# the-lay/voltools

Hardware: AMD Instinct MI355X
Metric: Mvoxels/s, 512^3 f32 filt_bspline StaticVolume transform (resident source, device output) (higher is better)
Workload: dtype f32; 1 GPU; 512^3 float32 filt_bspline, StaticVolume resident in HBM, rotate((0,i,0)) rzxz sweep, output= device buffer; lds_bytes=34816, kernel=8, resident_bytes=1660944384, angles=i

## Files before the change

### voltools_amd/csrc/vt_host.h

```cpp
#pragma once
#include "vt_internal.h"
#include "vt_resident.h"

#include <algorithm>
#include <cstdlib>
#include <vector>

struct Tuning {
    int tile = -1;
    int la = 0;
    int march_box = -1;
    int lxpad = -1;
    int dch = 0;
    int blk_h = -1, blk_w = -1;
    bool plain_tile_order = false;
    int rswap_wfast = -1;
    bool exp_nostore = false;
    bool exp_noload = false;
    bool exp_nolds = false;
    bool exp_noloop = false;
    bool exp_stamps = false;
    bool exp_notiles = false;
    bool exp_static = false;
    int quad_rows = -2;
    int quad_grid2d = 1;
    int quad_reverse = -1;
    bool test_fail_copy = false;
    int quad_perm = 1;
    bool no_proj_cache = false;
    int quad_pingpong = 1;
    int quad_zid = 1;
    int reorient = 4;
    int rows_pd = 8;
    int no_fused_relayout = 0;
    int rows_db = 0;
    int rows = 1;
    int quad_zfir = 1;
    int zid_dch = 0;
    int quad_nt = -1;
    bool no_block = false;
    int block_rs = -1;
    bool block_linear = false;
    bool block_no_trim = false;
    int block_min = 240;
    int block_pad = -1;
    double max_resident_gb = 0.0;
    int span = 1;
    int span_pipe = 0;
    int block_th = 8;
    int64_t dot_part_cap = 64ll << 20;
    void read()
    {
        auto num = [](const char* name, int dflt) { const char* e = std::getenv(name); return e ? std::atoi(e) : dflt; };
        tile = num("VT_TILE", -1);
#ifdef VT_LEGACY
        la = num("VT_LA", 0);
        march_box = num("VT_MARCH_BOX", -1);
        if (march_box > 1) march_box = 1;
        lxpad = num("VT_LXPAD", -1);
#endif
        dch = std::max(0, num("VT_DCH", 0));
        blk_h = num("VT_BLK_H", -1);
        blk_w = num("VT_BLK_W", -1);
        plain_tile_order = num("VT_TILE_ORDER", 1) == 0;
        rswap_wfast = num("VT_RSWAP_WFAST", -1);
#ifdef VT_EXPERIMENTS
        exp_nostore = std::getenv("VT_EXP_NOSTORE") != nullptr;
        exp_noload = std::getenv("VT_EXP_NOLOAD") != nullptr;
        exp_nolds = std::getenv("VT_EXP_NOLDS") != nullptr;
        exp_noloop = std::getenv("VT_EXP_NOLOOP") != nullptr;
        exp_static = std::getenv("VT_EXP_STATIC") != nullptr;
        exp_notiles = std::getenv("VT_EXP_NOTILES") != nullptr;
        exp_stamps = std::getenv("VT_EXP_STAMPS") != nullptr;
#endif
        quad_nt = num("VT_QUAD_NT", -1);
#ifdef VT_LEGACY
        test_fail_copy = std::getenv("VT_TEST_FAIL_COPY") != nullptr;
        quad_perm = num("VT_QUAD_PERM", 1);
        quad_zid = num("VT_QUAD_ZID", 1);
        quad_grid2d = num("VT_QUAD_GRID2D", 1);
#endif
        quad_pingpong = num("VT_QUAD_PINGPONG", 1);
        quad_zfir = num("VT_QUAD_ZFIR", 1);
        rows = num("VT_ROWS", 1);
        rows_pd = num("VT_ROWS_PD", 8);
        rows_db = num("VT_ROWS_DB", 0);
        no_fused_relayout = num("VT_NO_FUSED_RELAYOUT", 0);
        reorient = num("VT_REORIENT", 4);
        no_proj_cache = std::getenv("VT_NO_PROJ_CACHE") != nullptr;
        zid_dch = num("VT_ZID_DCH", 0);
        quad_reverse = num("VT_QUAD_REVERSE", -1);
        quad_rows = num("VT_QUAD_ROWS", -2);
        no_block = std::getenv("VT_NO_BLOCK_KERNEL") != nullptr;
        block_rs = num("VT_BLOCK_RS", -1);
        block_linear = std::getenv("VT_BLOCK_LINEAR") != nullptr;
        block_pad = num("VT_BLOCK_PAD", -1);
        block_th = num("VT_BLOCK_TH", 8) == 16 ? 16 : 8;
        span_pipe = num("VT_SPAN_PIPE", 0);
        span = num("VT_SPAN", 1);
        { const char* e = std::getenv("VT_MAX_RESIDENT_GB"); max_resident_gb = e ? std::atof(e) : 0.0; }
        block_min = std::max(1, num("VT_BLOCK_MIN", 240));
        block_no_trim = std::getenv("VT_BLOCK_NO_TRIM") != nullptr;
        { const char* e = std::getenv("VT_DOT_PART_CAP"); if (e && std::atoll(e) > 0) dot_part_cap = std::min<int64_t>(std::atoll(e), 64ll << 20); }
    }
};


struct vt_volume {
    unsigned launch_no = 0;
    int dev = 0;
    int interp = 0;
    int D = 0, H = 0, W = 0;
    int oD = 0, oH = 0, oW = 0;
    int64_t plane0 = 0;
    int64_t gD = 0;
    int64_t out_plane0 = 0;
    int P = 0;
    float* d_src = nullptr;
    size_t src_bytes = 0;
    float* d_zeros = nullptr;
    int Pr = 0;
    int Px = 0;
    int reorient_asked[3] = {0, 0, 0};
    vt::LazyCopies lazy;
    float copies_ms = 0.f;
    int copies_built = 0, copies_evicted = 0;
    hipEvent_t evc0 = nullptr, evc1 = nullptr;
    int* d_queue = nullptr;
    void* d_tplan = nullptr;
    size_t tplan_bytes = 0;
    uint32_t tplan_epoch = 0;
    float* d_scratch_out = nullptr;
    double* d_batch_m = nullptr;
    std::vector<double> h_batch_m;
    size_t batch_m_cap = 0;
    float* d_proj_tmp = nullptr;
    size_t proj_tmp_elems = 0;
    double* d_proj_part = nullptr;
    size_t proj_part_bytes = 0;
    vt_volume* proj = nullptr;
    bool proj_sum_valid = false;
    double proj_sum_m3 = 0.0;
    int proj_sum_oD = 0;
    int64_t proj_sum_oplane0 = 0;
    int edge_pad = 0;
    bool stack = false;
    bool owns_stream = true;
    bool deferred = false;
    bool lo_interior = false;
    size_t scratch_elems = 0;
    hipStream_t stream = nullptr;
    hipEvent_t ev0 = nullptr, ev1 = nullptr;
// ... 19 lines not shown
```

### voltools_amd/csrc/vt_internal.h

```cpp
#pragma once
#include <hip/hip_runtime.h>
#include <math.h>
#include <stdint.h>
#include "../../include/voltools_hip.h"

namespace vt {

constexpr float kPole   = -0x1.126148p-2f;
constexpr float kLambda =  0x1.7ffffep+2f;
constexpr float kAntiInit = 0x1.b0cb1ap-3f;

struct AffineParams {
    double m[12];
    double neg[3];
    double pos[3];
    double vlo[3];
    double vhi[3];
    int32_t inc_hi[3];
    uint32_t inc_lo[3];
    int32_t sD, sH, sW;
    int32_t sP;
    int32_t oD, oH, oW;
    int32_t nTd, nTh, nTw;
    int32_t Lz, Ly, Lx;
// ... 30 lines not shown
__host__ __device__ inline bool march_row_span(double a1, double b1, double a2, double b2, double ia1, double ib1,
                                               double by, double bx, int Y, int TH, int TW, int halo, int* mn, int* mx)
{
    const double ylo = (double)(Y - 1 - halo), yhi = (double)(Y + halo + 1);
    const double jm = (double)(TH - 1), km = (double)(TW - 1);
    double smin = 1e30, smax = -1e30;
    for (int cj = 0; cj < 2; ++cj)
        for (int ck = 0; ck < 2; ++ck) {
            const double j = cj ? jm : 0.0, k = ck ? km : 0.0;
            const double sy = by + a1 * j + b1 * k;
            if (sy >= ylo - 1e-6 && sy <= yhi + 1e-6) {
                const double sx = bx + a2 * j + b2 * k;
                smin = sx < smin ? sx : smin;
                smax = sx > smax ? sx : smax;
            }
        }
    for (int e = 0; e < 2; ++e) {
        const double L = e ? yhi : ylo;
        for (int c = 0; c < 2; ++c) {
            if (ib1 != 0.0) {
                const double j = c ? jm : 0.0;
                const double k = (L - by - a1 * j) * ib1;
                if (k >= 0.0 && k <= km) {
                    const double sx = bx + a2 * j + b2 * k;
                    smin = sx < smin ? sx : smin;
                    smax = sx > smax ? sx : smax;
                }
            }
            if (ia1 != 0.0) {
                const double k = c ? km : 0.0;
                const double j = (L - by - b1 * k) * ia1;
                if (j >= 0.0 && j <= jm) {
                    const double sx = bx + a2 * j + b2 * k;
                    smin = sx < smin ? sx : smin;
                    smax = sx > smax ? sx : smax;
                }
            }
        }
    }
    if (!(smin <= smax)) { *mn = 0; *mx = -1; return false; }
    *mn = (int)floor(smin - 1e-6) - halo;
    *mx = (int)floor(smax + 1e-6) + 1 + halo;
    return true;
}

struct PackGeom {
    double inv[9];
    double cst[3];
    double ext[3];
    int32_t T[3];
    int32_t halo;
    int32_t Lxbox;
    int32_t Lybox;
};

struct TilePlan {
    int kind;
    int cfg;
    int td, th, tw;
    int lds_bytes;
    int grid;
    int blocks_per_cu;
    PackGeom geo;
};

__host__ __device__ inline bool packed_row_span(const PackGeom& g, int Z, int Y, int* mn, int* mx)
{
    const double zlo = (double)(Z - 2 - 2 * g.halo) - 1e-6, zhi = (double)(Z + 1) + 1e-6;
    const double ylo = (double)(Y - 2 - 2 * g.halo) - 1e-6, yhi = (double)(Y + 1) + 1e-6;
    if (zhi < 0.0 || zlo > g.ext[0] || yhi < 0.0 || ylo > g.ext[1]) { *mn = 0; *mx = -1; return false; }
    double LB = 0.0, UB = g.ext[2];
    for (int c = 0; c < 3; ++c) {
        const double gz = g.inv[3 * c], gy = g.inv[3 * c + 1], gx = g.inv[3 * c + 2];
        if (gx > -1e-9 && gx < 1e-9) continue;
        const double inv_gx = 1.0 / gx;
        const double top = (double)(g.T[c] - 1);
        double lo_min = 1e30, hi_max = -1e30;
        for (int k = 0; k < 4; ++k) {
            const double uz = (k & 1) ? zhi : zlo, uy = (k & 2) ? yhi : ylo;
            const double s = gz * uz + gy * uy + g.cst[c];
            const double xa = (0.0 - s) * inv_gx, xb = (top - s) * inv_gx;
            const double lo = xa < xb ? xa : xb, hi = xa < xb ? xb : xa;
            lo_min = lo < lo_min ? lo : lo_min;
            hi_max = hi > hi_max ? hi : hi_max;
        }
        LB = lo_min > LB ? lo_min : LB;
        UB = hi_max < UB ? hi_max : UB;
    }
    if (LB > UB + 1e-6) { *mn = 0; *mx = -1; return false; }
    int a = (int)floor(LB - 1e-6);
    int b = (int)floor(UB + 1e-6 + (double)g.halo + 4.0) + 1 + g.halo;
    if (a < 0) a = 0;
    if (b > g.Lxbox - 1) b = g.Lxbox - 1;
    *mn = a;
    *mx = b;
    return a <= b;
}

struct ProjectParams {
    int32_t D, H;
    int32_t nxv;
    int32_t vec;
    int32_t src_pitch;
    int32_t dst_pitch;
    int64_t dst_plane;
    int32_t copies;
    int32_t uniform;
    int32_t zoff, halo, ntap;
    int32_t dlo, dhi;
    float wz[4];
};
hipError_t launch_plane_sum(const float* src, float* dst, const ProjectParams& q, hipStream_t stream);

int tile_config_count();
void tile_config(int idx, int* td, int* th, int* tw);
hipError_t launch_affine_tiled(int cfg, int interp, bool zsep, const float* src, float* out, const float* zeros16,
                               const AffineParams& p, int grid, int lds_bytes, hipStream_t stream);
hipError_t launch_affine_direct_batch(int interp, const float* src, float* out, const double* d_ms, int n,
                                      const AffineParams& p, hipStream_t stream);
int march_table_bytes();
int march_config_count();
void march_config(int idx, int* th, int* tw, int* g, int* la, int* nt);
int zpair_config_count();
void zpair_config(int idx, int* th, int* tw, int* la, int* nt);
int march_blocks_per_cu(bool pair, int cfg, int interp, int lds_bytes);
hipError_t launch_affine_zpair(int cfg, int interp, const float* src2, float* out, const AffineParams& p,
                               int grid, int lds_bytes, hipStream_t stream);
hipError_t launch_relayout_zpair(const float* src, float* dst, int D, int H, int W, int P, int P2, hipStream_t stream);
hipError_t launch_transpose02(const float* src, float* dst, int n0, int n1, int n2, int64_t ss0, int64_t ss1,
                              int64_t ds0, int64_t ds1, hipStream_t stream);
hipError_t launch_mirror_pad(const float* src, float* dst, int D, int H, int W, int R, int P, hipStream_t stream);
hipError_t launch_relayout_swap01(const float* src, float* dst, int D, int H, int P, hipStream_t stream);
int quad_max_it();
int quad_config_count();
void quad_config(int idx, int* th, int* tw, int* nt);
int quad_tile_plan_granules(int cfg);
int quad_tile_plan_lds(int cfg);
int quad_blocks_per_cu(int cfg, int interp, int lds_bytes, bool zid = false);
hipError_t init_quad_kernels();
hipError_t launch_relayout_zquad(const float* src, float* dst, int D, int H, int W, int P, int Pq, hipStream_t stream);
hipError_t launch_relayout_xfir(const float* src, float* dst, int D, int H, int W, int P, bool simple, hipStream_t stream);
hipError_t init_rows_kernels();
void rows_tile(int* ph, int* run);
hipError_t launch_affine_rows(int interp, int pd, const float* src, float* out, const float* zeros16, const AffineParams& p, int lds_bytes, hipStream_t stream);
// ... 105 lines not shown
```

### voltools_amd/csrc/vt_kernels_span.hip

```cpp
#include "vt_internal.h"
#include "vt_device.h"

namespace vt {

constexpr int kSpanMaxIt = 16;
constexpr int kSpanRowsMax = 1024;

typedef int v4i __attribute__((ext_vector_type(4)));
typedef float tap2 __attribute__((ext_vector_type(2), aligned(4)));

#pragma clang diagnostic push
#pragma clang diagnostic ignored "-Winline-asm"
__device__ __forceinline__ void span_dma16(int voff, v4i rs, unsigned m0v)
{
    asm volatile("s_mov_b32 m0, %2\n\ts_nop 0\n\tbuffer_load_dwordx4 %0, %1, 0 offen lds" : : "v"(voff), "s"(rs), "s"(m0v) : "memory", "m0");
}
__device__ __forceinline__ void span_dma16_global(const float* g, unsigned m0v)
{
    asm volatile("s_mov_b32 m0, %1\n\ts_nop 0\n\tglobal_load_lds_dwordx4 %0, off" : : "v"(g), "s"(m0v) : "memory", "m0");
}
#pragma clang diagnostic pop

__device__ __forceinline__ int queue_fetch_async(int* counter)
{
    typedef __attribute__((address_space(1))) int* global_int_ptr;
    global_int_ptr g = (global_int_ptr)counter;
    asm volatile("" : "+v"(g));
    return __hip_atomic_fetch_add(g, 1, __ATOMIC_RELAXED, __HIP_MEMORY_SCOPE_AGENT);
}

__device__ __forceinline__ int to_scalar(int v)
{
    asm volatile("" : "+v"(v));
    return __builtin_amdgcn_readfirstlane(v);
}

__device__ __forceinline__ uint64_t fx64(double x)
{
    const double fl = floor(x);
    double fr = rint((x - fl) * 4294967296.0);
    int hi = (int)fl;
    if (fr >= 4294967296.0) { fr = 0.0; hi += 1; }
    return ((uint64_t)(uint32_t)hi << 32) | (uint32_t)fr;
}
constexpr double kSpanOriginMargin = 4.0e-9;

template <int TD, bool MASKED, int UNROLL = 1>
__device__ __forceinline__ void span_gather_column(uint64_t c0, uint64_t c1, uint64_t c2, uint64_t inc0, uint64_t inc1, uint64_t inc2,
                                                   unsigned tbl_b, int Ly, __amdgpu_buffer_rsrc_t orsrc, int obj, int oplane_b, unsigned am, unsigned zm,
                                                   bool no_stores = false, bool no_lds = false, unsigned bdelta = 0u)
{
    typedef float v2f __attribute__((ext_vector_type(2)));
    int soff = 0;
#pragma unroll UNROLL
    for (int i0 = 0; i0 < TD; i0 += 4) {
        v4i t[4];
        unsigned xo[4];
        float fz[4], fy[4], fx[4];
#pragma unroll
        for (int u = 0; u < 4; ++u) {
            const int iz = (int)(c0 >> 32), iy = (int)(c1 >> 32);
            const unsigned ix = (unsigned)(c2 >> 32);
            const unsigned ta = tbl_b + 16u * (unsigned)(__mul24(iz, Ly) + iy);
            if (no_lds) t[u] = (v4i)((int)ta);
            else t[u] = *reinterpret_cast<const __attribute__((address_space(3))) v4i*>((size_t)ta);
            xo[u] = 4u * ix + bdelta;
            fz[u] = (float)(uint32_t)c0 * 0x1p-32f;
            fy[u] = (float)(uint32_t)c1 * 0x1p-32f;
            fx[u] = (float)(uint32_t)c2 * 0x1p-32f;
            c0 += inc0; c1 += inc1; c2 += inc2;
            asm("" : "+v"(c0), "+v"(c1), "+v"(c2));
        }
        tap2 a[4][4];
#pragma unroll
        for (int u = 0; u < 4; ++u) {
#pragma unroll
            for (int k = 0; k < 4; ++k) {
                if (no_lds) { a[u][k].x = fz[u] + (float)k; a[u][k].y = fy[u]; }
                else a[u][k] = *reinterpret_cast<const __attribute__((address_space(3))) tap2*>((size_t)((unsigned)t[u][k] + xo[u]));
            }
        }
#pragma unroll
        for (int u = 0; u < 4; ++u) {
            const v2f a00 = {a[u][0].x, a[u][0].y}, a01 = {a[u][1].x, a[u][1].y};
            const v2f a10 = {a[u][2].x, a[u][2].y}, a11 = {a[u][3].x, a[u][3].y};
            const v2f y0 = __builtin_elementwise_fma((v2f)(fy[u]), a01 - a00, a00);
            const v2f y1 = __builtin_elementwise_fma((v2f)(fy[u]), a11 - a10, a10);
            const v2f zz = __builtin_elementwise_fma((v2f)(fz[u]), y1 - y0, y0);
            const float val = fmaf(fx[u], zz.y - zz.x, zz.x);
            if constexpr (!MASKED) {
                if (!no_stores || val == 123.456f)
                    __builtin_amdgcn_raw_buffer_store_b32(__builtin_bit_cast(unsigned, val), orsrc, obj, soff + u * oplane_b, 0);
            } else {
                const bool sv = (am >> u) & 1u, sz = (zm >> u) & 1u;
                if (sv || sz) __builtin_amdgcn_raw_buffer_store_b32(sv ? __builtin_bit_cast(unsigned, val) : 0u, orsrc, obj, soff + u * oplane_b, 0);
            }
        }
        soff += 4 * oplane_b;
        if constexpr (MASKED) { am >>= 4; zm >>= 4; }
    }
}

template <int TD, int TH, int TW>
__global__ __launch_bounds__(256, 4) void affine_span(const float* __restrict__ src, float* __restrict__ out, const float* __restrict__ zeros16,
                                                      int* __restrict__ queue, const AffineParams p, const PackGeom geo)
{
    static_assert(256 % TW == 0 && TH % (256 / TW) == 0 && TD % 4 == 0, "tile/thread mapping");
    constexpr int RP = 256 / TW;
    constexpr int NJ = TH / RP;
    extern __shared__ __attribute__((aligned(16))) float lds[];

#ifdef VT_EXPERIMENTS
    const bool no_stores = (p.flags & (1 << 21)) != 0, no_loads = (p.flags & (1 << 22)) != 0, no_lds = (p.flags & (1 << 26)) != 0;
    const bool no_loop = (p.flags & (1 << 27)) != 0, static_ids = (p.flags & (1 << 28)) != 0;
    const bool no_tiles = (p.flags & (1 << 30)) != 0;
    const bool stamps = (p.flags & (1 << 29)) != 0;
    uint64_t st_acc[16] = {0, 0, 0, 0, 0, 0, 0, 0, 0, 0, 0, 0, 0, 0, 0, 0};
    int st_rim = 0, st_cnt[3] = {0, 0, 0};
    uint64_t st_prev = __builtin_amdgcn_s_memtime();
    const uint64_t st_begin = st_prev;
#define VT_STAMP(k) if (stamps) { const uint64_t now_ = __builtin_amdgcn_s_memtime(); st_acc[(k) + st_rim] += now_ - st_prev; st_prev = now_; }
#else
#define VT_STAMP(k)
    constexpr bool no_stores = false, no_loads = false, no_lds = false, no_loop = false, static_ids = false, no_tiles = false;
#endif
    const int tid = threadIdx.x;
    const int lane = tid & 63, wave = tid >> 6;
    const int wave_first = __builtin_amdgcn_readfirstlane(tid & ~63);
    const int Lz = p.Lz, Ly = p.Ly;
    const int rows = Lz * Ly;
    int* const tbl = reinterpret_cast<int*>(lds);
    int* const ctrl = tbl + 4 * rows;
    float* const buf = lds + p.slot_floats;
    const unsigned tbl_b = lds_byte_address(lds), buf_b = lds_byte_address(buf);

    int nv[4], x0s[4];
    int local = 0;
#pragma unroll
    for (int r = 0; r < 4; ++r) {
        const int row = tid * 4 + r;
        int mn = 0, mx = -1;
        const bool used = (row < rows) && packed_row_span(geo, row / Ly, row % Ly, &mn, &mx);
        x0s[r] = used ? (mn & ~3) : 0;
        nv[r] = used ? (((mx - x0s[r]) >> 2) + 1) : 0;
        local += nv[r];
    }
    const int incl = wave_scan_add(local);
    if (lane == 63) ctrl[wave] = incl;
    __syncthreads();
    int wave_off = 0;
#pragma unroll
    for (int w = 0; w < 4; ++w) wave_off += (w < wave) ? ctrl[w] : 0;
    const int nvec = ctrl[0] + ctrl[1] + ctrl[2] + ctrl[3];
    const int nvec_pad = (nvec + 63) & ~63;
    {
        int run = wave_off + incl - local;
#pragma unroll
        for (int r = 0; r < 4; ++r) {
            const int row = tid * 4 + r;
            if (row < rows) { tbl[4 * row] = run; tbl[4 * row + 1] = x0s[r]; }
            run += nv[r];
        }
    }
    const bool fits = (nvec_pad * 4 <= p.Lx) && (nvec_pad <= 256 * kSpanMaxIt);
    unsigned short* const vrow = reinterpret_cast<unsigned short*>(buf);
    if (fits) {
        int first = wave_off + incl - local;
#pragma unroll
        for (int r = 0; r < 4; ++r) {
            const int row = tid * 4 + r;
            for (int i = 0; i < nv[r]; ++i) vrow[first + i] = (unsigned short)row;
            first += nv[r];
        }
    }
    __syncthreads();
    int rel[kSpanMaxIt];
#pragma unroll
    for (int it = 0; it < kSpanMaxIt; ++it) {
        const int v = tid + 256 * it;
        const bool real = fits && v < nvec;
        const int row = real ? vrow[v] : 0;
        const int Z = row / Ly, Y = row - Z * Ly;
        const int xv = real ? tbl[4 * row + 1] + 4 * (v - tbl[4 * row]) : 0;
        rel[it] = real ? ((Z * p.sH + Y) * p.sP + xv) * 4 : -1;
    }
    __syncthreads();
    {
        v4i e[4];
#pragma unroll
        for (int r = 0; r < 4; ++r) {
            const int row = tid * 4 + r;
            e[r] = (v4i)(0);
            if (row < rows) {
                auto addr = [&](int rr) { return (int)buf_b + 4 * (4 * tbl[4 * rr] - tbl[4 * rr + 1]); };
                const int y = row % Ly;
                const int r01 = (y + 1 < Ly) ? row + 1 : row, r10 = (row + Ly < rows) ? row + Ly : row;
                const int r11 = (y + 1 < Ly && row + Ly < rows) ? row + Ly + 1 : r10;
                e[r] = (v4i){addr(row), addr(r01), addr(r10), addr(r11)};
            }
        }
        __syncthreads();
#pragma unroll
        for (int r = 0; r < 4; ++r) {
            const int row = tid * 4 + r;
            if (row < rows) *reinterpret_cast<v4i*>(tbl + 4 * row) = e[r];
        }
    }

    const int kw = tid % TW, jh0 = tid / TW;
    uint64_t coff[NJ][3];
    int ob[NJ];
#pragma unroll
    for (int jj = 0; jj < NJ; ++jj) {
        const int j = jh0 + jj * RP;
#pragma unroll
        for (int r = 0; r < 3; ++r) coff[jj][r] = fx64(fma(p.m[4 * r + 1], (double)j, p.m[4 * r + 2] * (double)kw));
        ob[jj] = (j * p.oW + kw) * 4;
    }
    const uint64_t inc0 = ((uint64_t)(uint32_t)p.inc_hi[0] << 32) | p.inc_lo[0];
    const uint64_t inc1 = ((uint64_t)(uint32_t)p.inc_hi[1] << 32) | p.inc_lo[1];
    const uint64_t inc2 = ((uint64_t)(uint32_t)p.inc_hi[2] << 32) | p.inc_lo[2];
    const int64_t ostride = (int64_t)p.oH * p.oW;
    const int oplane_b = (int)(ostride * 4);
    const bool keep = (p.flags & VT_KEEP_OUTSIDE) != 0;
    VT_STAMP(0)

    const bool plain_order = (p.flags & (1 << 23)) != 0;
    const int ntiles = p.nTd * p.nTh * p.nTw;
    const int nids = plain_order ? ntiles : blocked_tile_count(p.nTd, p.nTh, p.nTw);
    const int nSh = (p.nTh + 3) >> 2, nSw = (p.nTw + 3) >> 2;
    const int xcd = blockIdx.x & 7, per = (((nids + 63) >> 6) + 7) / 8 * 64;
    const int id0 = xcd * per, id_cnt = no_tiles ? 0 : max(0, min(per, nids - id0));
    int* const counter = queue + 32 * xcd;
    int nxt = 0;
    __syncthreads();
    const int nper = (int)gridDim.x >> 3, mine = (int)blockIdx.x >> 3;
    if (tid == 0) {
        if (static_ids) { ctrl[0] = mine; nxt = mine + nper; }
        else { ctrl[0] = atomicAdd(counter, 1); nxt = queue_fetch_async(counter); }
    }
    __syncthreads();
    int par = 0;
    if (!fits) {
        for (;;) {
            const int cur = ctrl[par];
            if (cur >= id_cnt) break;
            par ^= 1;
            int td_i, th_i, tw_i;
            const bool tile_ok = plain_order ? (td_i = (id0 + cur) / (p.nTh * p.nTw), th_i = ((id0 + cur) / p.nTw) % p.nTh, tw_i = (id0 + cur) % p.nTw, true)
                                             : blocked_tile(id0 + cur, p.nTd, p.nTh, p.nTw, td_i, th_i, tw_i);
            if (tile_ok) {
                const int d0 = td_i * TD, h0 = th_i * TH, w0 = tw_i * TW;
#pragma unroll 1
                for (int jj = 0; jj < NJ; ++jj) {
                    const int h = h0 + jh0 + jj * RP, w = w0 + kw;
                    if (h >= p.oH || w >= p.oW) continue;
                    const int nd = min(TD, p.oD - d0);
#pragma unroll 1
                    for (int i = 0; i < nd; ++i) {
                        const int d = d0 + i;
                        float* optr = out + ((int64_t)d * p.oH + h) * p.oW + w;
                        if (canonical_inside(p, d, h, w)) {
                            double sc[3];
#pragma unroll
                            for (int r = 0; r < 3; ++r) sc[r] = canonical_coord(p, r, d, h, w);
                            const double fzd = floor(sc[0]), fyd = floor(sc[1]), fxd = floor(sc[2]);
                            *optr = direct_sample<0>(src, p, (int)fzd, (int)fyd, (int)fxd, (float)(sc[0] - fzd), (float)(sc[1] - fyd), (float)(sc[2] - fxd));
                        } else if (!keep) *optr = 0.0f;
                    }
                }
            }
            if (tid == 0) { ctrl[par] = nxt; nxt = atomicAdd(counter, 1); }
            __syncthreads();
        }
    } else
    for (;;) {
// ... 1 lines not shown
        if (cur >= id_cnt) break;
        par ^= 1;
        typedef const __attribute__((address_space(4))) char* KArg;
        KArg ka = (KArg)__builtin_amdgcn_kernarg_segment_ptr();
        asm volatile("" : "+s"(ka));
        const auto* const kp = (const __attribute__((address_space(4))) AffineParams*)(ka + 32);
        const auto* const kg = (const __attribute__((address_space(4))) PackGeom*)(ka + 32 + sizeof(AffineParams));
        int mode = 0;
        bool fast = false, whole = false;
        int d0 = 0, h0 = 0, w0 = 0;
        uint64_t bfx[3] = {0, 0, 0};
        unsigned inm[NJ], zm[NJ];
#pragma unroll
        for (int jj = 0; jj < NJ; ++jj) { inm[jj] = 0xffffffffu; zm[jj] = 0u; }
        __amdgpu_buffer_rsrc_t orsrc = __builtin_amdgcn_make_buffer_rsrc(reinterpret_cast<char*>(out), 0, 0, 0x00020000);
        do {
            const int t = id0 + cur;
            int td_i, th_i, tw_i;
            bool tile_ok = true;
            if (plain_order) {
                tw_i = t % kp->nTw;
                const int t2 = t / kp->nTw;
                th_i = t2 % kp->nTh;
                td_i = t2 / kp->nTh;
            } else {
                const unsigned sbi = (unsigned)t >> 6, l6 = (unsigned)t & 63u;
                const unsigned s2 = nSw == 1 ? sbi : __umulhi(sbi, kp->nTw_magic), sbw = sbi - s2 * (unsigned)nSw;
                const unsigned sbd = nSh == 1 ? s2 : __umulhi(s2, kp->nTh_magic), sbh = s2 - sbd * (unsigned)nSh;
                td_i = (int)(sbd * 4 + (l6 >> 4)); th_i = (int)(sbh * 4 + ((l6 >> 2) & 3)); tw_i = (int)(sbw * 4 + (l6 & 3));
                tile_ok = td_i < kp->nTd && th_i < kp->nTh && tw_i < kp->nTw;
            }
            if (!tile_ok) break;
            d0 = td_i * TD; h0 = th_i * TH; w0 = tw_i * TW;
            VT_STAMP(1)

            double base[3], lo[3];
            bool any_valid = true, all_valid = true;
#pragma unroll
            for (int r = 0; r < 3; ++r) {
                base[r] = fma(kp->m[4 * r], (double)d0, fma(kp->m[4 * r + 1], (double)h0, fma(kp->m[4 * r + 2], (double)w0, kp->m[4 * r + 3])));
                lo[r] = base[r] + kp->neg[r];
                const double hi = base[r] + kp->pos[r];
                any_valid = any_valid && (hi >= kp->vlo[r] - kTileMargin) && (lo[r] < kp->vhi[r] + kTileMargin);
                all_valid = all_valid && (lo[r] >= kp->vlo[r] + kTileMargin) && (hi < kp->vhi[r] - kTileMargin);
            }
            whole = (d0 + TD <= kp->oD) && (h0 + TH <= kp->oH) && (w0 + TW <= kp->oW);
            const int64_t otile = (int64_t)d0 * ostride + (int64_t)h0 * kp->oW + w0;
            orsrc = __builtin_amdgcn_make_buffer_rsrc(reinterpret_cast<char*>(out + otile), 0, 0x7fffffff, 0x00020000);
            mode = 1;
            if (!any_valid) break;
            mode = 2;

            const int o0 = to_scalar((int)floor(lo[0] - kSpanOriginMargin)), o1 = to_scalar((int)floor(lo[1] - kSpanOriginMargin)),
                      o2 = to_scalar((int)floor(lo[2] - kSpanOriginMargin)) & ~3;
            const bool box_inside = o0 >= 0 && o1 >= 0 && o2 >= 0 && o0 + Lz <= kp->sD && o1 + Ly <= kp->sH && o2 + kg->Lxbox <= kp->sP;
            const int64_t origin = ((int64_t)o0 * kp->sH + o1) * kp->sP + o2;
            VT_STAMP(2)
#ifdef VT_EXPERIMENTS
            st_rim = (all_valid && whole && box_inside) ? 0 : 8;
            st_cnt[st_rim ? 1 : 0] += 1;
#endif

            const unsigned m0v = buf_b + 16u * (unsigned)wave_first;
            if (box_inside) {
                const uint64_t sb = (uint64_t)(size_t)(src + origin);
                const v4i rs = {(int)(uint32_t)sb, (int)((uint32_t)(sb >> 32) & 0xffffu), 0x7fffffff, 0x00020000};
#pragma unroll
                for (int it = 0; it < kSpanMaxIt; ++it) {
                    if (wave_first + 256 * it < nvec_pad && !no_loads)
                        span_dma16(max(rel[it], 0), rs, m0v + 4096u * it);
                }
            } else {
                const int row_f = kp->sP, plane_f = kp->sH * row_f;
                const float inv_row = 1.0f / (float)row_f, inv_plane = 1.0f / (float)plane_f;
#pragma unroll 1
                for (int it = 0; it < kSpanMaxIt; ++it) {
                    if (wave_first + 256 * it >= nvec_pad) break;
                    int r4 = rel[it];
                    asm volatile("" : "+v"(r4));
                    const int u = r4 >> 2;
                    int Z = (int)((float)u * inv_plane);
                    int rem = u - Z * plane_f;
                    if (rem < 0) { --Z; rem += plane_f; }
                    if (rem >= plane_f) { ++Z; rem -= plane_f; }
                    int Y = (int)((float)rem * inv_row);
                    int xv = rem - Y * row_f;
                    if (xv < 0) { --Y; xv += row_f; }
                    if (xv >= row_f) { ++Y; xv -= row_f; }
                    const int gz = o0 + Z, gy = o1 + Y, gx = o2 + xv;
                    const bool inb = r4 >= 0 && (unsigned)gz < (unsigned)kp->sD && (unsigned)gy < (unsigned)kp->sH && (unsigned)gx < (unsigned)kp->sP;
                    const float* g = inb ? reinterpret_cast<const float*>(reinterpret_cast<const char*>(src + origin) + r4) : zeros16;
                    span_dma16_global(g, m0v + 4096u * it);
                }
            }
            VT_STAMP(3)

            bfx[0] = fx64(base[0] - (double)o0);
            bfx[1] = fx64(base[1] - (double)o1);
            bfx[2] = fx64(base[2] - (double)o2);

            fast = all_valid && whole;
            if (!fast) {
                auto inside_canonical = [&](int d, int h, int w) {
                    const int c0 = kp->ord[0], c1 = kp->ord[1], c2 = kp->ord[2];
                    const double x0 = (double)(c0 == 0 ? d : (c0 == 1 ? h : w));
                    const double x1 = (double)(c1 == 0 ? d : (c1 == 1 ? h : w));
                    const double x2 = (double)(c2 == 0 ? d : (c2 == 1 ? h : w));
                    bool in = true;
#pragma unroll
                    for (int r = 0; r < 3; ++r) {
                        const double sc = fma(kp->m[4 * r + c0], x0, fma(kp->m[4 * r + c1], x1, fma(kp->m[4 * r + c2], x2, kp->m[4 * r + 3])));
                        in = in && (sc >= kp->vlo[r]) && (sc < kp->vhi[r]);
                    }
                    return in;
                };
#pragma unroll
                for (int jj = 0; jj < NJ; ++jj) {
                    const int h = h0 + jh0 + jj * RP, w = w0 + kw;
                    unsigned a = 0u, z = 0u;
                    if (h < kp->oH && w < kp->oW) {
                        const int nd = min(TD, kp->oD - d0);
#pragma unroll 1
                        for (int i = 0; i < nd; ++i) {
                            const bool inside = all_valid || inside_canonical(d0 + i, h, w);
                            a |= inside ? (1u << i) : 0u;
                            z |= (!inside && !keep) ? (1u << i) : 0u;
                        }
                    }
                    inm[jj] = a; zm[jj] = z;
                }
            }
            VT_STAMP(4)
            asm volatile("s_waitcnt vmcnt(0)" ::: "memory");
        } while (false);

        if (tid == 0) {
            ctrl[par] = nxt;
            if (static_ids) nxt += nper; else nxt = queue_fetch_async(counter);
        }
        if (mode == 2) {
            __syncthreads();
            VT_STAMP(5)
#pragma unroll
            for (int jj = 0; jj < NJ; ++jj) {
                const uint64_t c0 = bfx[0] + coff[jj][0], c1 = bfx[1] + coff[jj][1], c2 = bfx[2] + coff[jj][2];
                if (no_loop) { if (c0 == 12345u) out[c1] = 0.f; }
                else if (fast) span_gather_column<TD, false>(c0, c1, c2, inc0, inc1, inc2, tbl_b, Ly, orsrc, ob[jj], oplane_b, 0u, 0u, no_stores, no_lds);
                else span_gather_column<TD, true>(c0, c1, c2, inc0, inc1, inc2, tbl_b, Ly, orsrc, ob[jj], oplane_b, inm[jj], zm[jj]);
            }
            VT_STAMP(6)
        } else if (mode == 1) {
            if (!keep && !no_stores) {
#pragma unroll
                for (int jj = 0; jj < NJ; ++jj) {
                    const int h = h0 + jh0 + jj * RP, w = w0 + kw;
                    if (whole || (h < kp->oH && w < kp->oW)) {
                        const int nd = min(TD, kp->oD - d0);
                        for (int i = 0; i < nd; ++i) __builtin_amdgcn_raw_buffer_store_b32(0u, orsrc, ob[jj], i * oplane_b, 0);
                    }
                }
            }
            VT_STAMP(7)
#ifdef VT_EXPERIMENTS
            st_cnt[2] += 1;
#endif
        }
#ifdef VT_EXPERIMENTS
        st_rim = 0;
#endif
        __syncthreads();
        VT_STAMP(1)
    }
#ifdef VT_EXPERIMENTS
    if (stamps && tid == 0) {
        float* dbg = out + 16 * (size_t)blockIdx.x;
        for (int k = 0; k < 8; ++k) dbg[k] = (float)st_acc[k];
        dbg[8] = (float)(__builtin_amdgcn_s_memtime() - st_begin);
        for (int k = 3; k < 7; ++k) dbg[6 + k] = (float)st_acc[8 + k];
        dbg[13] = (float)st_cnt[0]; dbg[14] = (float)st_cnt[1]; dbg[15] = (float)st_cnt[2];
    }
#endif
    if (tid == 0) {
        __threadfence();
        if (atomicAdd(&queue[256], 1) == (int)gridDim.x - 1) {
#pragma unroll
            for (int i = 0; i < 9; ++i) queue[32 * i] = 0;
        }
    }
}

constexpr int kSpanWsMaxIt = 40;

template <int TD, int TH, int TW>
__global__ __launch_bounds__(320) void affine_span_ws(const float* __restrict__ src, float* __restrict__ out, const float* __restrict__ zeros16,
                                                      int* __restrict__ queue, const AffineParams p, const PackGeom geo)
{
    static_assert(TH * TW == 256 && TD % 4 == 0, "one column per consumer thread");
    extern __shared__ __attribute__((aligned(16))) float lds[];
    const int tid = threadIdx.x;
    const int lane = tid & 63, wave = tid >> 6;
    const bool producer = __builtin_amdgcn_readfirstlane(wave) == 4;
// ... 382 lines not shown
```

### voltools_amd/csrc/vt_plan.hip

```cpp
#include "vt_host.h"
#include "vt_device.h"

#include <cmath>
#include <cstring>

namespace vt {
namespace {

struct PlanCtx {
    const vt_volume* v;
    const double* m;
    int flags;
    AffineParams* p;
    TilePlan* plan;
    bool cubic;
    bool zsep;
    int halo2;
};

#ifdef VT_LEGACY
int64_t round_aware_chunks(int64_t oD, int g, int64_t inplane, int64_t resident, int64_t n0, int extra, int min_dch, int64_t n_floor)
{
    if (resident <= 0 || inplane > resident || inplane * n0 >= 16 * resident) return n0;
    auto cost = [&](int64_t n) {
// ... 543 lines not shown
    if (grid > 0x7fffffffLL) return false;
    plan->grid = (int)grid;
    return true;
}

struct PackedChoice { TilePlan plan; AffineParams p; double bpv; bool found; };

bool invert3(const double m[12], double inv[9])
{
    const double A[9] = {m[0], m[1], m[2], m[4], m[5], m[6], m[8], m[9], m[10]};
    const double det = A[0] * (A[4] * A[8] - A[5] * A[7]) - A[1] * (A[3] * A[8] - A[5] * A[6]) + A[2] * (A[3] * A[7] - A[4] * A[6]);
    double amax = 0;
    for (double a : A) amax = std::max(amax, std::fabs(a));
    if (!(std::fabs(det) > 1e-6 * amax * amax * amax && amax < 64.0)) return false;
    const double id = 1.0 / det;
    const double r[9] = {(A[4] * A[8] - A[5] * A[7]) * id, (A[2] * A[7] - A[1] * A[8]) * id, (A[1] * A[5] - A[2] * A[4]) * id,
                         (A[5] * A[6] - A[3] * A[8]) * id, (A[0] * A[8] - A[2] * A[6]) * id, (A[2] * A[3] - A[0] * A[5]) * id,
                         (A[3] * A[7] - A[4] * A[6]) * id, (A[1] * A[6] - A[0] * A[7]) * id, (A[0] * A[4] - A[1] * A[3]) * id};
    for (int i = 0; i < 9; ++i) inv[i] = r[i];
    return true;
}

void pick_packed_tile(PlanCtx& c, const double inv[9], PackedChoice* out)
{
    const vt_volume* v = c.v;
    const double* m = c.m;
    double best = 1e300;
    out->found = false;
    const bool span = !c.cubic && v->tune.span != 0;
    const int ncfg = span ? span_config_count() : packed_config_count();
    for (int cfg = 0; cfg < ncfg; ++cfg) {
        if (v->tune.tile >= 0 && cfg != v->tune.tile) continue;
        int T[3];
        if (span) span_config(cfg, &T[0], &T[1], &T[2]); else packed_config(cfg, &T[0], &T[1], &T[2]);
        const int64_t tiles_c = (int64_t)((v->oD + T[0] - 1) / T[0]) * ((v->oH + T[1] - 1) / T[1]) * ((v->oW + T[2] - 1) / T[2]);
        if (!(c.flags & VT_FORCE_PACKED) && tiles_c < 6 * (int64_t)v->cu_count * (c.cubic ? 2 : 3)) continue;
        PackGeom g;
        int L[3];
        bool ok = true;
        double neg[3], pos[3];
        for (int r = 0; r < 3 && ok; ++r) {
            double ext = 0;
            neg[r] = pos[r] = 0;
            for (int k = 0; k < 3; ++k) {
                const double e = m[4 * r + k] * (T[k] - 1);
                ext += std::fabs(e);
                if (e < 0) neg[r] += e; else pos[r] += e;
            }
            if (!(ext < 1000.0)) { ok = false; break; }
            g.ext[r] = ext;
            L[r] = (int)std::floor(ext + (span ? 1.0e-8 : 0.0)) + 3 + c.halo2;
        }
        if (!ok) continue;
        L[2] = (L[2] + 3 + 3) & ~3;
        const int rows = L[0] * L[1];
        if (rows > (span ? span_rows_max() : packed_rows_max()) || L[2] > 4000 || L[1] > 1023 || L[0] > 511) continue;
        if ((int64_t)L[0] * v->H * v->P * 4 >= 0x7fffffffLL) continue;
        if (span && (int64_t)(T[0] + 1) * v->oH * v->oW * 4 >= 0x7fffffffLL) continue;
        if (span && (L[1] > v->H || L[2] > v->P)) continue;
        for (int i = 0; i < 9; ++i) g.inv[i] = inv[i];
        for (int cc = 0; cc < 3; ++cc) g.cst[cc] = inv[3 * cc] * neg[0] + inv[3 * cc + 1] * neg[1] + inv[3 * cc + 2] * neg[2];
        g.T[0] = T[0]; g.T[1] = T[1]; g.T[2] = T[2];
        g.halo = c.cubic ? 1 : 0;
        g.Lxbox = L[2];
        g.Lybox = L[1];
        int nvec = 0;
        for (int row = 0; row < rows; ++row) {
            int mn, mx;
            if (packed_row_span(g, row / L[1], row % L[1], &mn, &mx)) nvec += ((mx - (mn & ~3)) >> 2) + 1;
        }
        int cap_vec = nvec + rows / 16 + 8;
        if (span) cap_vec = (cap_vec + 63) & ~63;
        if (cap_vec > (span ? span_vectors_max() : packed_vectors_max())) continue;
        const bool pipe = span && span_config_pipelined(cfg);
        if (span && v->tune.span_pipe >= 0 && pipe != (v->tune.span_pipe != 0)) continue;
        if (pipe && cap_vec > 2560) continue;
        const int table_floats = span ? (pipe ? 4 * rows + 84 : 4 * rows + 8) : (2 * rows + 8 + 3) & ~3;
        const int64_t bytes = ((int64_t)table_floats + (int64_t)cap_vec * 4 * (pipe ? 2 : 1) + (pipe ? cap_vec : 0)) * 4;
        if (bytes > v->lds_limit) continue;
        const int blocks_per_cu = (int)std::min<int64_t>(c.cubic ? 2 : (span ? 4 : 3), (160 * 1024) / bytes);
        const double vox = (double)T[0] * T[1] * T[2];
        double cost = (double)bytes / vox * (blocks_per_cu >= 3 ? 1.0 : (blocks_per_cu == 2 ? 1.2 : 2.0));
        if (span) cost *= (blocks_per_cu >= 4 ? 0.90 : 1.0) * (T[0] >= 16 ? 1.0 : 1.15) * (T[2] >= 32 ? 0.93 : 1.0);
        if (cost < best) {
            best = cost;
            out->found = true;
            out->bpv = (double)(((int64_t)table_floats + (int64_t)cap_vec * 4) * 4) / vox;
            out->plan.kind = 6; out->plan.cfg = cfg; out->plan.td = T[0]; out->plan.th = T[1]; out->plan.tw = T[2];
            out->plan.lds_bytes = (int)bytes;
            out->p.Lz = L[0]; out->p.Ly = L[1]; out->p.Lx = cap_vec * 4;
            out->p.slot_floats = table_floats;
            for (int r = 0; r < 3; ++r) { out->p.neg[r] = neg[r]; out->p.pos[r] = pos[r]; }
            out->plan.geo = g;
            out->plan.blocks_per_cu = blocks_per_cu;
        }
    }
}

bool plan_packed(PlanCtx& c, bool have_box, double box_bpv)
{
    const vt_volume* v = c.v;
    if (c.zsep || (c.flags & VT_NO_PACKED) || (c.cubic && !(c.flags & VT_FORCE_PACKED))) return false;
    double inv[9];
    if (!invert3(c.m, inv)) return false;
    PackedChoice pk;
    pk.plan = *c.plan;
    pk.p = *c.p;
    pick_packed_tile(c, inv, &pk);
    if (!pk.found) return false;
    const bool forced = (c.flags & VT_FORCE_PACKED) != 0;
    const int64_t pk_tiles = (int64_t)((v->oD + pk.plan.td - 1) / pk.plan.td) * ((v->oH + pk.plan.th - 1) / pk.plan.th) *
                             ((v->oW + pk.plan.tw - 1) / pk.plan.tw);
    const bool enough = pk_tiles >= 6 * (int64_t)v->cu_count * std::max(1, pk.plan.blocks_per_cu);
    const bool beyond_cache = (int64_t)v->D * v->H * v->P * 4 > (256LL << 20);
    const double margin = c.cubic ? 0.5 : (beyond_cache ? 1.0 : 0.6);
    if (!(!have_box || forced || (enough && pk.bpv < margin * box_bpv))) return false;
    *c.plan = pk.plan;
    *c.p = pk.p;
    AffineParams* p = c.p;
    p->nTd = (v->oD + pk.plan.td - 1) / pk.plan.td;
    p->nTh = (v->oH + pk.plan.th - 1) / pk.plan.th;
    p->nTw = (v->oW + pk.plan.tw - 1) / pk.plan.tw;
    const int64_t ntiles = (int64_t)p->nTd * p->nTh * p->nTw;
    if (ntiles > 0x7fffffffLL) { c.plan->kind = 1; return true; }
    if (v->tune.plain_tile_order) p->flags |= (1 << 23);
    p->flags |= experiment_flags(v);
    int64_t nwg = std::min<int64_t>(ntiles, (int64_t)v->cu_count * std::max(1, c.plan->blocks_per_cu));
    nwg = std::max<int64_t>(8, (nwg + 7) / 8 * 8);
    c.plan->grid = (int)nwg;
    p->dch = 1;
// ... 56 lines not shown
    }
    const int lx_used = (L[2] + 3 + 3) & ~3;
    int rs_idx = -1, RS = 0, PS = 0;
    int64_t vectors = 0;
    auto try_rs = [&](int idx) {
        if (idx < 0 || idx >= block_rs_count() || (th == 16 && idx > 2) || block_rs(idx) < lx_used) return false;
        const int rs = block_rs(idx);
        int best_pad = 0;
        double best_f = 1e300;
        for (int pad = 0; pad < 64; pad += 4) {
            if ((int64_t)L[0] * (L[1] * rs + pad) / 4 > block_max_vectors(th)) break;
            const double f = block_conflicts(m, 0, rs, L[1] * rs + pad, c.cubic) * (1.0 + 0.002 * pad);
            if (f < best_f - 1e-9) { best_f = f; best_pad = pad; }
        }
        if (v->tune.block_pad >= 0) best_pad = v->tune.block_pad & ~3;
        const int ps = L[1] * rs + best_pad;
        const int64_t vec = (int64_t)L[0] * ps / 4;
        if (vec > block_max_vectors(th)) return false;
        rs_idx = idx; RS = rs; PS = ps; vectors = vec;
        return true;
    };
    if (v->tune.block_rs >= 0) {
        if (!try_rs(v->tune.block_rs)) return false;
    } else {
        const int* order = nullptr;
        const int norder = block_rs_order(th, &order);
        bool ok = false;
        for (int i = 0; i < norder && !ok; ++i) ok = try_rs(order[i]);
        if (!ok) return false;
    }
    const int64_t plane_b = (int64_t)v->H * v->P * 4;
    if ((int64_t)L[0] * plane_b >= 0x7fffffffLL || (int64_t)T[0] * v->oH * v->oW * 4 >= 0x7fffffffLL) return false;
    const int box_bytes = (int)((vectors + 63) / 64 * 64 * 16);
    const int lds_bytes = box_bytes + 16;
    if (lds_bytes > v->lds_limit) return false;

    plan->kind = 9; plan->cfg = rs_idx; plan->td = T[0]; plan->th = T[1]; plan->tw = T[2];
    plan->lds_bytes = lds_bytes;
    p->Lz = L[0]; p->Ly = L[1]; p->Lx = RS; p->Lx_used = lx_used; p->Lps = PS;
    p->flags = (c.flags & VT_KEEP_OUTSIDE) | experiment_flags(v);
    set_tile_reach(p, m, T, 0);
    double inv[9];
    if (!v->tune.block_no_trim && invert3(m, inv)) {
        PackGeom& g = plan->geo;
        for (int i = 0; i < 9; ++i) g.inv[i] = inv[i];
        for (int cc = 0; cc < 3; ++cc) g.cst[cc] = inv[3 * cc] * p->neg[0] + inv[3 * cc + 1] * p->neg[1] + inv[3 * cc + 2] * p->neg[2];
        for (int r = 0; r < 3; ++r) {
            g.ext[r] = p->pos[r] - p->neg[r];
            g.T[r] = T[r];
        }
        g.halo = c.cubic ? 1 : 0;
        g.Lxbox = lx_used;
        g.Lybox = L[1];
        p->flags |= (1 << 25);
    }
    p->nTd = (v->oD + T[0] - 1) / T[0];
    p->nTh = (v->oH + T[1] - 1) / T[1];
    p->nTw = (v->oW + T[2] - 1) / T[2];
    p->psv_magic = (uint32_t)(4294967296.0 / (double)(PS / 4)) + 1u;
    p->lds_cap = box_bytes;
    p->nTw_magic = (uint32_t)((1ULL << 32) / (uint64_t)((p->nTw + 3) >> 2) + 1);
    p->nTh_magic = (uint32_t)((1ULL << 32) / (uint64_t)((p->nTh + 3) >> 2) + 1);
    const int col[5] = {2, 1, 2, 0, 1};
    const double mul[5] = {8.0, 8.0, -8.0, 4.0, -8.0};
    const int neg_of[5] = {-1, -1, 0, -1, 1};
    for (int s = 0; s < 5; ++s)
        for (int r = 0; r < 3; ++r) {
            if (neg_of[s] >= 0) {
                const uint64_t fwd = ((uint64_t)(uint32_t)p->binc_hi[neg_of[s]][r] << 32) | p->binc_lo[neg_of[s]][r];
                const uint64_t back = 0 - fwd;
                p->binc_hi[s][r] = (int32_t)(uint32_t)(back >> 32); p->binc_lo[s][r] = (uint32_t)back;
                continue;
            }
            const double step = m[4 * r + col[s]] * mul[s];
            const double fl = std::floor(step);
            double lo = std::floor((step - fl) * 4294967296.0 + 0.5);
            int32_t hi = (int32_t)fl;
            if (lo >= 4294967296.0) { lo = 0; hi += 1; }
            p->binc_hi[s][r] = hi; p->binc_lo[s][r] = (uint32_t)lo;
        }
    plan->blocks_per_cu = (int)std::min<int64_t>(th == 16 ? 2 : 4, (160 * 1024) / lds_bytes);
    const int64_t ids = blocked_tile_count(p->nTd, p->nTh, p->nTw);
    int64_t grid = std::min<int64_t>((int64_t)v->cu_count * plan->blocks_per_cu, ids);
    grid = std::max<int64_t>(8, (grid + 7) / 8 * 8);
    p->dch = (int)std::max<int64_t>(1, std::min<int64_t>(4, ids / (grid * 8)));
    plan->grid = (int)grid;
    return true;
}

bool plan_general(PlanCtx& c)
{
    double box_bpv = 1e300;
    const bool have_box = pick_box_tile(c, &box_bpv);
    if (plan_packed(c, have_box, box_bpv)) return true;
    if (!have_box) return false;
    const double* mm = c.m;
    const double det = mm[0] * (mm[5] * mm[10] - mm[6] * mm[9]) - mm[1] * (mm[4] * mm[10] - mm[6] * mm[8]) + mm[2] * (mm[4] * mm[9] - mm[5] * mm[8]);
    if (c.plan->kind == 2 && !(c.flags & VT_FORCE_TILED) && c.v->tune.tile < 0 && std::fabs(det) >= 9.0 &&
        (c.plan->lds_bytes > 80 * 1024 || (!c.cubic && box_bpv > 43.0))) {
        c.plan->kind = 1; c.plan->cfg = -1; c.plan->td = c.plan->th = c.plan->tw = 0; c.plan->lds_bytes = 0; c.plan->grid = 0;
        return true;
    }
    if (!finish_box(c)) { c.plan->kind = 1; }
    return true;
}

// ... 140 lines not shown
```

Measured before the change: 704,800 Mvoxels/s.

## Pack span row table into 16-bit offsets and allow unaligned tight x spans

Shrinks the per-row LDS lookup table of the non-pipelined span kernel from four 32-bit entries to two 32-bit words holding four 16-bit biased offsets. The gather loads 8 bytes instead of 16 and unpacks them. An optional tight mode (VT_SPAN_ALIGN=0) drops the 4-alignment of row x-starts, adding a scalar fallback load for vectors that straddle the volume edge. This cuts LDS footprint and table-read bandwidth, which may raise occupancy or allow larger tiles, at the cost of unpack instructions and new 16-bit range limits on the buffer size.

```diff
diff --git a/voltools_amd/csrc/vt_host.h b/voltools_amd/csrc/vt_host.h
--- a/voltools_amd/csrc/vt_host.h
+++ b/voltools_amd/csrc/vt_host.h
@@ -47,6 +47,7 @@
     double max_resident_gb = 0.0;
     int span = 1;
     int span_pipe = 0;
+    int span_align = 1;
     int block_th = 8;
     int64_t dot_part_cap = 64ll << 20;
     void read()
@@ -98,6 +99,7 @@
         block_th = num("VT_BLOCK_TH", 8) == 16 ? 16 : 8;
         span_pipe = num("VT_SPAN_PIPE", 0);
         span = num("VT_SPAN", 1);
+        span_align = num("VT_SPAN_ALIGN", 1);
         { const char* e = std::getenv("VT_MAX_RESIDENT_GB"); max_resident_gb = e ? std::atof(e) : 0.0; }
         block_min = std::max(1, num("VT_BLOCK_MIN", 240));
         block_no_trim = std::getenv("VT_BLOCK_NO_TRIM") != nullptr;
diff --git a/voltools_amd/csrc/vt_internal.h b/voltools_amd/csrc/vt_internal.h
--- a/voltools_amd/csrc/vt_internal.h
+++ b/voltools_amd/csrc/vt_internal.h
@@ -106,6 +106,7 @@
     int32_t halo;
     int32_t Lxbox;
     int32_t Lybox;
+    int32_t xslack;
 };
 
 struct TilePlan {
@@ -143,7 +144,7 @@
     }
     if (LB > UB + 1e-6) { *mn = 0; *mx = -1; return false; }
     int a = (int)floor(LB - 1e-6);
-    int b = (int)floor(UB + 1e-6 + (double)g.halo + 4.0) + 1 + g.halo;
+    int b = (int)floor(UB + 1e-6 + (double)g.xslack) + 1 + g.halo;
     if (a < 0) a = 0;
     if (b > g.Lxbox - 1) b = g.Lxbox - 1;
     *mn = a;
diff --git a/voltools_amd/csrc/vt_kernels_span.hip b/voltools_amd/csrc/vt_kernels_span.hip
--- a/voltools_amd/csrc/vt_kernels_span.hip
+++ b/voltools_amd/csrc/vt_kernels_span.hip
@@ -7,6 +7,7 @@
 constexpr int kSpanRowsMax = 1024;
 
 typedef int v4i __attribute__((ext_vector_type(4)));
+typedef unsigned v2u __attribute__((ext_vector_type(2)));
 typedef float tap2 __attribute__((ext_vector_type(2), aligned(4)));
 
 #pragma clang diagnostic push
@@ -45,7 +46,7 @@
 }
 constexpr double kSpanOriginMargin = 4.0e-9;
 
-template <int TD, bool MASKED, int UNROLL = 1>
+template <int TD, bool MASKED, int UNROLL = 1, int ENTRY = 16>
 __device__ __forceinline__ void span_gather_column(uint64_t c0, uint64_t c1, uint64_t c2, uint64_t inc0, uint64_t inc1, uint64_t inc2,
                                                    unsigned tbl_b, int Ly, __amdgpu_buffer_rsrc_t orsrc, int obj, int oplane_b, unsigned am, unsigned zm,
                                                    bool no_stores = false, bool no_lds = false, unsigned bdelta = 0u)
@@ -61,9 +62,13 @@
         for (int u = 0; u < 4; ++u) {
             const int iz = (int)(c0 >> 32), iy = (int)(c1 >> 32);
             const unsigned ix = (unsigned)(c2 >> 32);
-            const unsigned ta = tbl_b + 16u * (unsigned)(__mul24(iz, Ly) + iy);
+            const unsigned ta = tbl_b + (unsigned)ENTRY * (unsigned)(__mul24(iz, Ly) + iy);
             if (no_lds) t[u] = (v4i)((int)ta);
-            else t[u] = *reinterpret_cast<const __attribute__((address_space(3))) v4i*>((size_t)ta);
+            else if constexpr (ENTRY == 16) t[u] = *reinterpret_cast<const __attribute__((address_space(3))) v4i*>((size_t)ta);
+            else {
+                const v2u e = *reinterpret_cast<const __attribute__((address_space(3))) v2u*>((size_t)ta);
+                t[u] = (v4i){(int)(e.x & 0xffffu), (int)(e.x >> 16), (int)(e.y & 0xffffu), (int)(e.y >> 16)};
+            }
             xo[u] = 4u * ix + bdelta;
             fz[u] = (float)(uint32_t)c0 * 0x1p-32f;
             fy[u] = (float)(uint32_t)c1 * 0x1p-32f;
@@ -130,9 +135,10 @@
     const int Lz = p.Lz, Ly = p.Ly;
     const int rows = Lz * Ly;
     int* const tbl = reinterpret_cast<int*>(lds);
-    int* const ctrl = tbl + 4 * rows;
+    int* const ctrl = tbl + 2 * rows;
     float* const buf = lds + p.slot_floats;
     const unsigned tbl_b = lds_byte_address(lds), buf_b = lds_byte_address(buf);
+    const int xmask = (geo.xslack > geo.halo + 1) ? ~3 : ~0;
 
     int nv[4], x0s[4];
     int local = 0;
@@ -141,8 +147,10 @@
         const int row = tid * 4 + r;
         int mn = 0, mx = -1;
         const bool used = (row < rows) && packed_row_span(geo, row / Ly, row % Ly, &mn, &mx);
-        x0s[r] = used ? (mn & ~3) : 0;
+        x0s[r] = used ? (mn & xmask) : 0;
         nv[r] = used ? (((mx - x0s[r]) >> 2) + 1) : 0;
+        nv[r] = min(nv[r], geo.Lxbox >> 2);
+        if (x0s[r] + 4 * nv[r] > geo.Lxbox) x0s[r] = geo.Lxbox - 4 * nv[r];
         local += nv[r];
     }
     const int incl = wave_scan_add(local);
@@ -158,11 +166,12 @@
 #pragma unroll
         for (int r = 0; r < 4; ++r) {
             const int row = tid * 4 + r;
-            if (row < rows) { tbl[4 * row] = run; tbl[4 * row + 1] = x0s[r]; }
+            if (row < rows) { tbl[2 * row] = run; tbl[2 * row + 1] = x0s[r]; }
             run += nv[r];
         }
     }
-    const bool fits = (nvec_pad * 4 <= p.Lx) && (nvec_pad <= 256 * kSpanMaxIt);
+    const int bias_b = 4 * geo.Lxbox;
+    const bool fits = (nvec_pad * 4 <= p.Lx) && (nvec_pad <= 256 * kSpanMaxIt) && (16 * nvec_pad + bias_b <= 0xffff);
     unsigned short* const vrow = reinterpret_cast<unsigned short*>(buf);
     if (fits) {
         int first = wave_off + incl - local;
@@ -181,29 +190,30 @@
         const bool real = fits && v < nvec;
         const int row = real ? vrow[v] : 0;
         const int Z = row / Ly, Y = row - Z * Ly;
-        const int xv = real ? tbl[4 * row + 1] + 4 * (v - tbl[4 * row]) : 0;
+        const int xv = real ? tbl[2 * row + 1] + 4 * (v - tbl[2 * row]) : 0;
         rel[it] = real ? ((Z * p.sH + Y) * p.sP + xv) * 4 : -1;
     }
     __syncthreads();
     {
-        v4i e[4];
+        unsigned e0[4], e1[4];
 #pragma unroll
         for (int r = 0; r < 4; ++r) {
             const int row = tid * 4 + r;
-            e[r] = (v4i)(0);
+            e0[r] = e1[r] = 0u;
             if (row < rows) {
-                auto addr = [&](int rr) { return (int)buf_b + 4 * (4 * tbl[4 * rr] - tbl[4 * rr + 1]); };
+                auto off = [&](int rr) { return (unsigned)(bias_b + 4 * (4 * tbl[2 * rr] - tbl[2 * rr + 1])); };
                 const int y = row % Ly;
                 const int r01 = (y + 1 < Ly) ? row + 1 : row, r10 = (row + Ly < rows) ? row + Ly : row;
                 const int r11 = (y + 1 < Ly && row + Ly < rows) ? row + Ly + 1 : r10;
-                e[r] = (v4i){addr(row), addr(r01), addr(r10), addr(r11)};
+                e0[r] = off(row) | (off(r01) << 16);
+                e1[r] = off(r10) | (off(r11) << 16);
             }
         }
         __syncthreads();
 #pragma unroll
         for (int r = 0; r < 4; ++r) {
             const int row = tid * 4 + r;
-            if (row < rows) *reinterpret_cast<v4i*>(tbl + 4 * row) = e[r];
+            if (row < rows) { tbl[2 * row] = (int)e0[r]; tbl[2 * row + 1] = (int)e1[r]; }
         }
     }
 
@@ -222,6 +232,7 @@
     const uint64_t inc2 = ((uint64_t)(uint32_t)p.inc_hi[2] << 32) | p.inc_lo[2];
     const int64_t ostride = (int64_t)p.oH * p.oW;
     const int oplane_b = (int)(ostride * 4);
+    const unsigned tap_base = buf_b - (unsigned)bias_b;
     const bool keep = (p.flags & VT_KEEP_OUTSIDE) != 0;
     VT_STAMP(0)
 
@@ -329,7 +340,7 @@
             mode = 2;
 
             const int o0 = to_scalar((int)floor(lo[0] - kSpanOriginMargin)), o1 = to_scalar((int)floor(lo[1] - kSpanOriginMargin)),
-                      o2 = to_scalar((int)floor(lo[2] - kSpanOriginMargin)) & ~3;
+                      o2 = to_scalar((int)floor(lo[2] - kSpanOriginMargin)) & xmask;
             const bool box_inside = o0 >= 0 && o1 >= 0 && o2 >= 0 && o0 + Lz <= kp->sD && o1 + Ly <= kp->sH && o2 + kg->Lxbox <= kp->sP;
             const int64_t origin = ((int64_t)o0 * kp->sH + o1) * kp->sP + o2;
             VT_STAMP(2)
@@ -365,9 +376,21 @@
                     if (xv < 0) { --Y; xv += row_f; }
                     if (xv >= row_f) { ++Y; xv -= row_f; }
                     const int gz = o0 + Z, gy = o1 + Y, gx = o2 + xv;
-                    const bool inb = r4 >= 0 && (unsigned)gz < (unsigned)kp->sD && (unsigned)gy < (unsigned)kp->sH && (unsigned)gx < (unsigned)kp->sP;
-                    const float* g = inb ? reinterpret_cast<const float*>(reinterpret_cast<const char*>(src + origin) + r4) : zeros16;
-                    span_dma16_global(g, m0v + 4096u * it);
+                    const bool row_in = r4 >= 0 && (unsigned)gz < (unsigned)kp->sD && (unsigned)gy < (unsigned)kp->sH;
+                    const bool cut = row_in && ((gx < 0 && gx + 4 > 0) || (gx < kp->sP && gx + 4 > kp->sP));
+                    if (!cut) {
+                        const bool inb = row_in && gx >= 0 && gx + 4 <= kp->sP;
+                        const float* g = inb ? reinterpret_cast<const float*>(reinterpret_cast<const char*>(src + origin) + r4) : zeros16;
+                        span_dma16_global(g, m0v + 4096u * it);
+                    } else {
+                        const float* const grow = src + ((int64_t)gz * kp->sH + gy) * kp->sP;
+                        float4 e;
+                        e.x = (unsigned)gx < (unsigned)kp->sP ? grow[gx] : 0.0f;
+                        e.y = (unsigned)(gx + 1) < (unsigned)kp->sP ? grow[gx + 1] : 0.0f;
+                        e.z = (unsigned)(gx + 2) < (unsigned)kp->sP ? grow[gx + 2] : 0.0f;
+                        e.w = (unsigned)(gx + 3) < (unsigned)kp->sP ? grow[gx + 3] : 0.0f;
+                        *reinterpret_cast<float4*>(buf + 4 * (tid + 256 * it)) = e;
+                    }
                 }
             }
             VT_STAMP(3)
@@ -422,8 +445,8 @@
             for (int jj = 0; jj < NJ; ++jj) {
                 const uint64_t c0 = bfx[0] + coff[jj][0], c1 = bfx[1] + coff[jj][1], c2 = bfx[2] + coff[jj][2];
                 if (no_loop) { if (c0 == 12345u) out[c1] = 0.f; }
-                else if (fast) span_gather_column<TD, false>(c0, c1, c2, inc0, inc1, inc2, tbl_b, Ly, orsrc, ob[jj], oplane_b, 0u, 0u, no_stores, no_lds);
-                else span_gather_column<TD, true>(c0, c1, c2, inc0, inc1, inc2, tbl_b, Ly, orsrc, ob[jj], oplane_b, inm[jj], zm[jj]);
+                else if (fast) span_gather_column<TD, false, 1, 8>(c0, c1, c2, inc0, inc1, inc2, tbl_b, Ly, orsrc, ob[jj], oplane_b, 0u, 0u, no_stores, no_lds, tap_base);
+                else span_gather_column<TD, true, 1, 8>(c0, c1, c2, inc0, inc1, inc2, tbl_b, Ly, orsrc, ob[jj], oplane_b, inm[jj], zm[jj], false, false, tap_base);
             }
             VT_STAMP(6)
         } else if (mode == 1) {
diff --git a/voltools_amd/csrc/vt_plan.hip b/voltools_amd/csrc/vt_plan.hip
--- a/voltools_amd/csrc/vt_plan.hip
+++ b/voltools_amd/csrc/vt_plan.hip
@@ -619,7 +619,10 @@
             L[r] = (int)std::floor(ext + (span ? 1.0e-8 : 0.0)) + 3 + c.halo2;
         }
         if (!ok) continue;
-        L[2] = (L[2] + 3 + 3) & ~3;
+        const bool pipe = span && span_config_pipelined(cfg);
+        if (span && v->tune.span_pipe >= 0 && pipe != (v->tune.span_pipe != 0)) continue;
+        const bool tight = span && !pipe && v->tune.span_align == 0;
+        L[2] = tight ? L[2] + 4 : (L[2] + 3 + 3) & ~3;
         const int rows = L[0] * L[1];
         if (rows > (span ? span_rows_max() : packed_rows_max()) || L[2] > 4000 || L[1] > 1023 || L[0] > 511) continue;
         if ((int64_t)L[0] * v->H * v->P * 4 >= 0x7fffffffLL) continue;
@@ -631,18 +634,24 @@
         g.halo = c.cubic ? 1 : 0;
         g.Lxbox = L[2];
         g.Lybox = L[1];
+        g.xslack = g.halo + (tight ? 1 : 4);
         int nvec = 0;
+        bool rows_inside = true;
         for (int row = 0; row < rows; ++row) {
             int mn, mx;
-            if (packed_row_span(g, row / L[1], row % L[1], &mn, &mx)) nvec += ((mx - (mn & ~3)) >> 2) + 1;
-        }
+            if (packed_row_span(g, row / L[1], row % L[1], &mn, &mx)) {
+                const int x0 = tight ? mn : (mn & ~3), n = ((mx - x0) >> 2) + 1;
+                nvec += n;
+                rows_inside = rows_inside && x0 >= 0 && x0 + 4 * n <= L[2];
+            }
+        }
+        if (!rows_inside) continue;
         int cap_vec = nvec + rows / 16 + 8;
         if (span) cap_vec = (cap_vec + 63) & ~63;
         if (cap_vec > (span ? span_vectors_max() : packed_vectors_max())) continue;
-        const bool pipe = span && span_config_pipelined(cfg);
-        if (span && v->tune.span_pipe >= 0 && pipe != (v->tune.span_pipe != 0)) continue;
         if (pipe && cap_vec > 2560) continue;
-        const int table_floats = span ? (pipe ? 4 * rows + 84 : 4 * rows + 8) : (2 * rows + 8 + 3) & ~3;
+        if (span && !pipe && (int64_t)cap_vec * 16 + 4 * L[2] > 0xffff) continue;
+        const int table_floats = span ? (pipe ? 4 * rows + 84 : (2 * rows + 8 + 3) & ~3) : (2 * rows + 8 + 3) & ~3;
         const int64_t bytes = ((int64_t)table_floats + (int64_t)cap_vec * 4 * (pipe ? 2 : 1) + (pipe ? cap_vec : 0)) * 4;
         if (bytes > v->lds_limit) continue;
         const int blocks_per_cu = (int)std::min<int64_t>(c.cubic ? 2 : (span ? 4 : 3), (160 * 1024) / bytes);
@@ -805,6 +814,7 @@
         g.halo = c.cubic ? 1 : 0;
         g.Lxbox = lx_used;
         g.Lybox = L[1];
+        g.xslack = g.halo + 4;
         p->flags |= (1 << 25);
     }
     p->nTd = (v->oD + T[0] - 1) / T[0];
```

New measurement: 704,300 Mvoxels/s, median of 3. About the same (-0.1%).
